# OmerShubi/DL_VQA

Measured on AMD Instinct MI355X. Metric: VQA samples/sec (train step), higher is better.
Workload: dtype f32; 1 GPU; VqaNet train step (fwd+softCE+bwd+Adam), batch 256/GPU, 224x224 images, 14-token questions, 1000-way head, train mode; global_batch=256, image_size=224, answers=1000, vocab=5000, parallelism=dp1

## Files before the change

dl_vqa_amd/_lib.py:

```python
from __future__ import annotations

import ctypes as C
import os

import torch

_HERE = os.path.dirname(os.path.abspath(__file__))
LIB_PATH = os.environ.get("VQA_LIB", os.path.join(_HERE, "libvqa_hip.so"))
HEADER_PATH = os.path.join(os.path.dirname(_HERE), "include", "vqa_hip.h")


def header_abi_version() -> int:
    import re
    with open(HEADER_PATH) as f:
        m = re.search(r"^#define\s+VQA_ABI_VERSION\s+(\d+)", f.read(), flags=re.M)
    if not m:
        raise VqaHipError(f"{HEADER_PATH}: no VQA_ABI_VERSION")
    return int(m.group(1))


f32p = C.c_void_p
u8p = C.c_void_p
i64p = C.c_void_p
i32, i64, f32, u64, vp = C.c_int, C.c_int64, C.c_float, C.c_uint64, C.c_void_p
# ... 86 lines not shown
    "vqa_preprocess_supported": (i32, [vp, vp, i64, i32, i32]),
    "vqa_preprocess_images": (i32, [u8p, i64, vp, vp, i64, vp, vp, i32, i32, vp, i32, vp, vp]),
    "vqa_f32_to_bf16": (i32, [f32p, vp, i64, vp]),
    "vqa_bf16_to_f32": (i32, [vp, f32p, i64, vp]),
    "vqa_dropout_to_bf16": (i32, [f32p, vp, i64, f32, u64, vp]),
    "vqa_f32_to_bf16_transpose": (i32, [f32p, vp, i32, i32, vp]),
    "vqa_gemm_bf16_workspace_bytes": (i64, [i32, i32, i32]),
    "vqa_gemm_bf16": (i32, [vp, i64, i32, vp, i64, i32, vp, i64, i32, i32, i32, i32, f32p, f32p,
                            f32p, i64, i32, i32, i32, i32, f32p, f32p, i64, i32, vp]),
    "vqa_gemm_plan": (i32, [i32, i32, i32, i32, i32, i32, i64, C.POINTER(i32), i32]),
    "vqa_gemm_tall_bf16_supported": (i32, [i32, i32, i32, i32, i32]),
    "vqa_gemm_tall_bf16_plan": (i32, [i32, i32, i32, C.POINTER(i32), i32]),
    "vqa_gemm_tall_bf16": (i32, [vp, i64, vp, i64, vp, i64, i32, i32, i32, f32p, i64, i32, i32, i32, i32, vp]),
    "vqa_conv_pack_weights_bf16": (i32, [f32p, vp, vp, i32, i32, i32, vp]),
    "vqa_conv3x3_relu_pool_fwd_bf16": (i32, [vp, vp, f32p, vp, i32, u8p, i32, i32, i32, i32, i32, i32, i32, vp]),
    "vqa_conv3x3_dgrad_bf16": (i32, [vp, u8p, vp, vp, i32, i32, i32, i32, i32, i32, i32, i32, vp]),
    "vqa_conv3x3_wgrad_bf16_workspace_bytes": (i64, [i32, i32, i32, i32, i32, i32]),
    "vqa_conv3x3_wgrad_bf16": (i32, [vp, vp, u8p, f32p, f32p, i32, i32, i32, i32, i32, i32, i32, f32p, i64, i32, vp]),
    "vqa_pconvf_supported": (i32, [i32, i32, i32, i32, i32]),
    "vqa_pconvf_weights_bytes": (i64, [i32, i32]),
    "vqa_pconvf_pack_weights": (i32, [f32p, f32p, i32, i32, vp]),
    "vqa_pconvf_dgrad": (i32, [f32p, u8p, f32p, f32p, i32, i32, i32, i32, i32, i32, vp]),
    "vqa_pconv_supported": (i32, [i32, i32, i32, i32, i32]),
    "vqa_pconv_weights_bytes": (i64, [i32, i32]),
    "vqa_pconv_pack_weights": (i32, [f32p, vp, vp, i32, i32, vp]),
    "vqa_pconv_fwd": (i32, [vp, vp, f32p, vp, i32, u8p, i32, i32, i32, i32, i32, i32, vp]),
    "vqa_pconv_wgrad_supported": (i32, [i32, i32, i32, i32]),
    "vqa_pconv_wgrad_workspace_bytes": (i64, [i32, i32, i32, i32, i32]),
    "vqa_pconv_wgrad": (i32, [vp, u8p, vp, f32p, f32p, i32, i32, i32, i32, i32, f32p, i64, i32, vp]),
    "vqa_pconv_dgrad": (i32, [vp, u8p, vp, vp, i32, i32, i32, i32, i32, i32, i32, vp]),
    "vqa_adam": (i32, [f32p, f32p, f32p, f32p, i64, f32, f32, f32, f32, i32, f32, vp]),
    "vqa_adam_segments": (i32, [f32p, f32p, f32p, f32p, i64, vp, i32, f32, vp]),
    "vqa_conv3x3_x3_plan": (i32, [i32, i32, i32, i32, i32, i32, i32, C.POINTER(i32), i32]),
}

K_GEMM, K_CONV_FWD, K_CONV_DGRAD, K_CONV_WGRAD = 0, 1, 2, 3
(K_L2NORM_FWD, K_L2NORM_BWD, K_ATT_SCORE_FWD, K_ATT_SCORE_BWD, K_ATT_APPLY_FWD, K_ATT_APPLY_BWD, K_ADAM, K_SOFTCE,
 K_DROPOUT, K_LSTM_SEQ, K_COUNT) = range(4, 15)


class LstmDir(C.Structure):
    _fields_ = [("w_hh", vp), ("xg", vp), ("gates", vp), ("Hs", vp), ("Cs", vp), ("c_final", vp),
                ("dgates", vp), ("dh", vp), ("dc", vp), ("reverse", i32)]


class AdamSegment(C.Structure):
    _fields_ = [("begin", i64), ("end", i64), ("lr", f32), ("beta1", f32), ("beta2", f32), ("eps", f32),
                ("weight_decay", f32), ("step", i32), ("decoupled", i32)]


ADAM_MAX_SEGMENTS = 64


class VqaHipError(RuntimeError):
    pass


_lib = None


def load() -> C.CDLL:
    global _lib
    if _lib is not None:
        return _lib
    if not os.path.exists(LIB_PATH):
        raise VqaHipError(
# ... 29 lines not shown
```

dl_vqa_amd/build.py:

```python
from __future__ import annotations

import os
import subprocess
import sys
from concurrent.futures import ThreadPoolExecutor

HERE = os.path.dirname(os.path.abspath(__file__))
CSRC = os.path.join(HERE, "csrc")
LIB = os.path.join(HERE, "libvqa_hip.so")
SOURCES = ([("gemm.hip", f"_p{k}", [f"-DVQA_GEMM_PART={k}"]) for k in (2, 3, 4, 5)]
           + [("gemm_x3.hip", f"_p{k}", [f"-DVQA_GEMM_PART={k}"]) for k in (1, 2, 3, 4)]
           + ["bf16.hip", ("gemm.hip", "_p1", ["-DVQA_GEMM_PART=1"]), "conv.hip", "conv_x3.hip", "conv_bf16.hip", "conv_patch_bf16.hip", "conv_patch_f32.hip", "gemm_tall_bf16.hip", "gemm.hip",
              "gemm_x3.hip", "runtime.hip", "conv0.hip", "conv0_dgrad.hip", "lstm.hip", "elementwise.hip", "conv_generic.hip", "att_score.hip", "topk.hip", "preprocess.hip"])
HEADERS = ["common.hpp", "gemm_core.hpp", "gemm_epilogue.hpp", "gemm_host.hpp", "bf16_core.hpp", "x3_core.hpp", "conv_device.inc", "conv_host.inc", "conv_bf16.inc", os.path.join("..", "..", "include", "vqa_hip.h")]
FLAGS = ["-O3", "--offload-arch=gfx950", "-fPIC", "-std=c++17", "-Wno-unused-result"]


def _hipcc() -> str:
    for cand in (os.environ.get("HIPCC"), "/opt/rocm/bin/hipcc", "hipcc"):
        if cand and (os.path.isabs(cand) and os.path.exists(cand) or not os.path.isabs(cand)):
            return cand
    return "hipcc"


def _stale(target: str, deps) -> bool:
    if not os.path.exists(target):
        return True
    t = os.path.getmtime(target)
    return any(os.path.getmtime(d) > t for d in deps if os.path.exists(d))


def _deps(src: str, seen=None) -> list:
    import re
    seen = set() if seen is None else seen
    out = []
    try:
        text = open(src).read()
    except OSError:
        return out
    for inc in re.findall(r'^\s*#\s*include\s+"([^"]+)"', text, flags=re.M):
        path = os.path.normpath(os.path.join(os.path.dirname(src), inc))
        if path not in seen and os.path.exists(path):
            seen.add(path)
            out.append(path)
            out += _deps(path, seen)
    return out
# ... 34 lines not shown
```

dl_vqa_amd/csrc/conv0.hip:

```cpp
#include "x3_core.hpp"

namespace vqa {

__host__ __device__ inline int c0_round_stride(int W, int want_mod) {
  int rs = W + 2;
  while (rs % 32 != want_mod) ++rs;
  return rs;
}

__device__ __forceinline__ float4 c0_load4(const void* x, int64_t e, int xh) {
  if (xh) {
    typedef _Float16 h16x4 __attribute__((ext_vector_type(4)));
    const h16x4 hv = *reinterpret_cast<const h16x4*>(static_cast<const uint16_t*>(x) + e);
    return make_float4((float)hv[0], (float)hv[1], (float)hv[2], (float)hv[3]);
  }
  return *reinterpret_cast<const float4*>(static_cast<const float*>(x) + e);
}

constexpr int C0_FR = 4;
constexpr int C0_PR = 2 * C0_FR + 2;

struct C0Tap { int c, ky, kx; };
__device__ __forceinline__ C0Tap c0_tap(int k) {
  const int c = k / 9, t = k - 9 * c, ky = t / 3;
// ... 644 lines not shown
#pragma unroll
      for (int j = 0; j < TN; ++j)
#pragma unroll
        for (int m = 0; m < 4; ++m) {
          const int o = (8 * g + 4 * h + m) * Co + 32 * j + l31;
          const uint32_t code = ams[o];
          const uint32_t dz = (uint32_t)dps[o] & ((code >> 2) - 1u);
          bsum[j] += __uint_as_float(dz << 16);
          const uint64_t f = (uint64_t)dz << ((code & 3u) * 16u);
          wlo[j][m] = (uint32_t)f;
          whi[j][m] = (uint32_t)(f >> 32);
        }
#pragma unroll
      for (int hs = 0; hs < 2; ++hs) {
        const bf16x8 af = __builtin_bit_cast(bf16x8, *reinterpret_cast<const uint4*>(arow + hs * RSTR + 32 * g));
#pragma unroll
        for (int j = 0; j < TN; ++j) {
          const bf16x8 bf = __builtin_bit_cast(bf16x8, hs ? make_uint4(whi[j][0], whi[j][1], whi[j][2], whi[j][3])
                                                          : make_uint4(wlo[j][0], wlo[j][1], wlo[j][2], wlo[j][3]));
          acc[j] = __builtin_amdgcn_mfma_f32_32x32x16_bf16(af, bf, acc[j], 0, 0, 0);
        }
      }
    }
  }
  c0_wgrad_write_slab<TN>(lds, acc, bsum, slab, bias_slab, tid, wave, l31, h);
}

__global__ void conv0_wgrad_reduce_kernel(const float* slab, const float* bias_slab, float* dw, float* dbias,
                                          int parts, int K, int Co) {
  __shared__ float red[256];
  const int k = blockIdx.x;
  const int co = threadIdx.x % Co, sl = threadIdx.x / Co, nsl = 256 / Co;
  float v = 0.f;
  if (sl < nsl)
    for (int p = sl; p < parts; p += nsl)
      v += (k < K) ? slab[((int64_t)p * 32 + k) * Co + co] : bias_slab[(int64_t)p * Co + co];
  red[threadIdx.x] = v;
  __syncthreads();
  if (sl == 0) {
    for (int s2 = 1; s2 < nsl; ++s2) v += red[s2 * Co + co];
    if (k < K) dw[(int64_t)co * K + k] = v; else dbias[co] = v;
  }
}

constexpr size_t kC0LdsMax = 160 * 1024;

static size_t c0_fwd_lds(int Ci, int W, int Co, bool wide_f32) {
  return (size_t)Ci * C0_PR * c0_round_stride(W, 16) * 4 + (wide_f32 ? (size_t)4 * 8 * Co * 5 : 0);
}
static int c0_c16_stride(int W) {
  int rs = W + 2;
  while (rs % 64 != 16) ++rs;
  return rs;
}
static size_t c0_fwd_c16_lds(int Ci, int W, int Co, int waves) {
  return (size_t)Ci * C0_PR * c0_c16_stride(W) * 2 + (size_t)waves * 8 * Co * 3 + (size_t)2 * (Co / 32) * 1024;
}
static int c0_wgrad_plane(int W) {
  int plane = 4 * c0_round_stride(W, 11);
  while (plane % 32 != 3) ++plane;
  return plane;
}
static size_t c0_combine_lds(int Co) { return (size_t)(4 * 32 + 4) * Co * 4; }
static size_t c0_wgrad_lds(int Ci, int W, int Co) {
  const size_t lds = (((size_t)Ci * c0_wgrad_plane(W) + 3) & ~(size_t)3) * 4 + (size_t)((W - 2) / 2) * Co * 5;
  return lds < c0_combine_lds(Co) ? c0_combine_lds(Co) : lds;
}
static size_t c0_wgrad_bf16_lds(int Ci, int RSTR, int NG, int Co) {
  const size_t lds = (size_t)3 * Ci * 4 * RSTR + (size_t)8 * NG * Co * 3;
// ... 145 lines not shown
```

dl_vqa_amd/csrc/elementwise.hip:

```cpp
#include <hip/hip_fp16.h>
#include "common.hpp"

namespace vqa {

__global__ void dropout_kernel(const float* x, float* y, int64_t n, float p, float inv_keep, uint64_t seed) {
  for (int64_t i = (int64_t)blockIdx.x * blockDim.x + threadIdx.x; i < n; i += (int64_t)gridDim.x * blockDim.x)
    y[i] = x[i] * drop_scale(seed, (uint64_t)i, p, inv_keep);
}

__global__ void dropout_add_kernel(const float* x, float* y, int64_t n, float p, float inv_keep, uint64_t seed) {
  const int64_t n4 = n / 4;
  for (int64_t i = (int64_t)blockIdx.x * blockDim.x + threadIdx.x; i < n4; i += (int64_t)gridDim.x * blockDim.x) {
    const float4 a = reinterpret_cast<const float4*>(x)[i];
    float4 b = reinterpret_cast<float4*>(y)[i];
    const float4 ds_ = drop_scale4(seed, (uint64_t)(4 * i), p, inv_keep);
    b.x += a.x * ds_.x; b.y += a.y * ds_.y; b.z += a.z * ds_.z; b.w += a.w * ds_.w;
    reinterpret_cast<float4*>(y)[i] = b;
  }
  if (blockIdx.x == 0 && threadIdx.x < n - 4 * n4) {
    const int64_t i = 4 * n4 + threadIdx.x;
    y[i] += x[i] * drop_scale(seed, (uint64_t)i, p, inv_keep);
  }
}

// ... 728 lines not shown
      float g = wsum * expf(row[i] - mx) * invs;
      for (int k = 0; k < kmax; ++k)
        if (a_idx[(int64_t)b * kmax + k] == (int64_t)i + 1) g -= (float)a_val[(int64_t)b * kmax + k] / 10.0f;
      d[i] = g * inv_batch;
    }
  }
}

__global__ void colsum_stage1(const float* x, int64_t ld, const uint8_t* mask, int64_t rows, int cols,
                              int64_t rows_per, float* slab) {
  __shared__ float part[4][64];
  const int cl = threadIdx.x & 63, rl = threadIdx.x >> 6;
  const int c = blockIdx.x * 64 + cl;
  const int64_t r0 = (int64_t)blockIdx.y * rows_per;
  const int64_t r1 = r0 + rows_per < rows ? r0 + rows_per : rows;
  float acc = 0.f;
  if (c < cols)
    for (int64_t r = r0 + rl; r < r1; r += 4) {
      const float v = x[r * ld + c];
      if (!mask || mask[r * cols + c] != 4) acc += v;
    }
  part[rl][cl] = acc;
  __syncthreads();
  if (rl == 0 && c < cols) slab[(int64_t)blockIdx.y * cols + c] = part[0][cl] + part[1][cl] + part[2][cl] + part[3][cl];
}
__global__ void colsum_stage2(const float* slab, int splits, int cols, float* out, int accumulate) {
  const int c = blockIdx.x * blockDim.x + threadIdx.x;
  if (c >= cols) return;
  float v = 0.f;
  for (int s = 0; s < splits; ++s) v += slab[(int64_t)s * cols + c];
  out[c] = accumulate ? out[c] + v : v;
}

static void colsum_plan(int64_t rows, int cols, int* splits, int64_t* rows_per) {
  const int ctiles = (cols + 63) / 64;
  int64_t s = (1024 + ctiles - 1) / ctiles;
  const int64_t max_s = (rows + 63) / 64;
  if (s > max_s) s = max_s;
  if (s < 1) s = 1;
  *rows_per = (rows + s - 1) / s;
  *splits = (int)((rows + *rows_per - 1) / *rows_per);
}
int64_t colsum_ws_bytes(int64_t rows, int cols) {
  int splits; int64_t rp;
  colsum_plan(rows, cols, &splits, &rp);
  return (int64_t)splits * cols * 4;
}
int colsum_launch(const float* x, int64_t ld, const uint8_t* mask, int64_t rows, int cols, float* out,
                  int accumulate, float* ws, int64_t ws_bytes, hipStream_t s) {
  int splits; int64_t rp;
  colsum_plan(rows, cols, &splits, &rp);
  if (!ws || ws_bytes < (int64_t)splits * cols * 4) {
    set_error("colsum: workspace %lld < %lld", (long long)ws_bytes, (long long)splits * cols * 4);
    return VQA_ERR_WORKSPACE;
  }
  hipLaunchKernelGGL(colsum_stage1, dim3((cols + 63) / 64, splits), dim3(256), 0, s, x, ld, mask, rows, cols, rp, ws);
  int rc = check_hip(hipGetLastError(), "colsum_stage1 launch");
  if (rc) return rc;
  hipLaunchKernelGGL(colsum_stage2, dim3((cols + 255) / 256), dim3(256), 0, s, ws, splits, cols, out, accumulate);
  return check_hip(hipGetLastError(), "colsum_stage2 launch");
}

__global__ __launch_bounds__(1024) void sum_bgp_kernel(const float* x, float* out, int B, int G, int P) {
  __shared__ float red[16];
  const int g = blockIdx.x;
  const int lane = threadIdx.x & 63, w = threadIdx.x >> 6;
  float s = 0.f;
// ... 571 lines not shown
```

dl_vqa_amd/csrc/gemm_core.hpp:

```cpp
#pragma once
#include <type_traits>
#include "common.hpp"

namespace vqa {

typedef float f32x16 __attribute__((ext_vector_type(16)));

#ifdef VQA_DIAG
static __device__ unsigned long long vqa_diag_buf[4];
static __device__ unsigned long long vqa_diag_ld[4];
#endif

#ifndef VQA_PRIO_MFMA
#define VQA_PRIO_MFMA 3
#endif
#ifndef VQA_EARLY_BARRIER
#define VQA_EARLY_BARRIER 2
#endif
#ifndef VQA_PF128
#define VQA_PF128 2
#endif
#ifndef VQA_PRIO_LOADER
#define VQA_PRIO_LOADER 0
#endif
// ... 567 lines not shown
}
template <class Cfg>
__device__ __forceinline__ int acc_col(int wn, int j, int lane) {
  return wn * Cfg::WN + 32 * j + (lane & 31);
}

template <class Cfg>
__device__ __forceinline__ void store_acc_tiles(f32x16 (&acc)[Cfg::TM][Cfg::TN], float* out, int64_t ld, int rows,
                                                int cols, int m0, int n0, int wm, int wn, int lane) {
  const bool interior = m0 + Cfg::BM <= rows && n0 + Cfg::BN <= cols;
  const uint32_t ldb = (uint32_t)ld * 4u;
  const uint32_t vl = (uint32_t)(4 * (lane >> 5)) * ldb + 4u * (uint32_t)(lane & 31);
  auto body = [&](auto inner) {
    constexpr bool INNER = decltype(inner)::value;
#pragma unroll
    for (int i = 0; i < Cfg::TM; ++i)
#pragma unroll
      for (int j = 0; j < Cfg::TN; ++j) {
        const int rowt = m0 + wm * Cfg::WM + 32 * i, colt = n0 + wn * Cfg::WN + 32 * j;
        const __amdgpu_buffer_rsrc_t rs = buf_rsrc(out + (int64_t)rowt * ld + colt);
        const bool cok = colt + (lane & 31) < cols;
#pragma unroll
        for (int r = 0; r < 16; ++r) {
          const int dr = (r & 3) + 8 * (r >> 2);
          const bool ok = INNER || (cok && rowt + 4 * (lane >> 5) + dr < rows);
          buf_store4(rs, acc[i][j][r], ok ? vl : BUF_OOB, (uint32_t)dr * ldb);
        }
      }
  };
  if (interior) body(std::true_type{}); else body(std::false_type{});
}

struct TileCoord { int mt, nt, split; };
__device__ __forceinline__ TileCoord tile_coord(int tiles_m, int tiles_n, int order = 0, int splits = 1) {
  const int t = xcd_swizzle(blockIdx.x, gridDim.x);
  const int tiles = tiles_m * tiles_n;
  TileCoord c;
  if (order == 1) {
    const int per_nt = tiles_m * splits;
    c.nt = t / per_nt;
    const int u = t - c.nt * per_nt;
    c.split = u / tiles_m;
    c.mt = u - c.split * tiles_m;
    return c;
  }
  c.split = t / tiles;
  const int u = t - c.split * tiles;
  c.mt = u / tiles_n;
  c.nt = u - c.mt * tiles_n;
  return c;
}

}
```

dl_vqa_amd/engine.py:

```python
from __future__ import annotations

import functools
import inspect
import os
from collections import namedtuple
from types import SimpleNamespace
from typing import Callable, Dict, Optional

import torch

from . import ops

Tensor = torch.Tensor

SITE_IMAGE, SITE_TEXT, SITE_ATT_V, SITE_ATT_Q, SITE_ATT_X, SITE_CLS1, SITE_CLS2 = 1, 2, 3, 4, 5, 6, 7
_MASK64 = (1 << 64) - 1


def _site_seed(base: int, site: int) -> int:
    return (base * 0x9E3779B97F4A7C15 + site * 0xD1B54A32D192ED03 + 0x632BE59BD9B4E019) & _MASK64


_SFX = ("", "_reverse")

# ... 492 lines not shown
                                                                   self.att_mode, ctx.p_att, sd(SITE_ATT_X))
        ops.colsum(dwx_part, n * NT, wx.numel(), Gr["attention.x_conv.weight"])
        dqp = new(B, mid)
        ops.sum_parts(dq_part, dqp, B, NT, mid)
        gx3 = self._x3_gemm(n * Pn)
        ops.gemm(dvprime, ctx.v_in, Gr["attention.v_conv.weight"], mid, C, n * Pn, transA=True, transB=False, lda=mid, ldb=C,
                 tag=44, x3=gx3)
        if encoded:
            dv_in = new(n * Pn, C)
            ops.gemm(dvprime, P["attention.v_conv.weight"], dv_in, n * Pn, C, mid, transB=False, lda=mid, ldb=C, tag=45, x3=gx3)
        self._q_lin_bwd(P, ctx, dqp, dcomb, Gr)
        ready("attention")

        def question_branch():
            self._question_bwd(P, ctx, dcomb, Gr)
            ready("text")

        if not encoded:
            question_branch()
            return None
        _, text_done = self._on_side_stream(dev, question_branch, backward=True)
        ops.dropout_add(dv_in, dvn, ctx.p_att, sd(SITE_ATT_V))
        dP = ops.l2norm_bwd(dvn, ctx.vn, ctx.norm, ctx.p_img, sd(SITE_IMAGE)).view_as(ctx.acts[-1])
        dv = self._conv_bwd(P, ctx, dP, Gr)
        ready("image")
        torch.cuda.current_stream(dev).wait_event(text_done)
        return dv

    @_device_current("dlogits")
    def backward(self, P: Dict[str, Tensor], ctx, dlogits: Tensor, Gr: Dict[str, Tensor],
                 on_ready: Optional[Callable[[str], None]] = None) -> Optional[Tensor]:
        dev = dlogits.device
        ready = on_ready if on_ready is not None else (lambda group: None)
        dcomb = self._classifier_bwd(P, ctx, dlogits, Gr)
        ready("classifier")
        dv_in = self._attention_bwd(P, ctx, dcomb, Gr)
        ready("attention")

        def question_branch():
            self._question_bwd(P, ctx, dcomb, Gr)
            ready("text")

        _, text_done = self._on_side_stream(dev, question_branch, backward=True)
        dv = self._image_bwd(P, ctx, dcomb, dv_in, Gr)
        ready("image")
        torch.cuda.current_stream(dev).wait_event(text_done)
        return dv

    def _classifier_bwd(self, P, ctx, dlogits, Gr):
        B, Dc, hid, A = ctx.B, self.Dc, self.hid, self.A
        dev = dlogits.device
        sd = lambda site: _site_seed(ctx.seed, site)
        if (A > 1 and dlogits.stride(1) != 1) or (B > 1 and dlogits.stride(0) < A):
            dlogits = dlogits.contiguous()
        ldA = (A + 3) // 4 * 4
        if ldA != A or not dlogits.is_contiguous() or dlogits.data_ptr() % 16:
            dl = torch.zeros(B, ldA, dtype=torch.float32, device=dev)
            ops.add2d(dlogits, dlogits.stride(0), None, 0, dl, ldA, B, A)
            dlogits = dl
        fc = ctx.fc
        if fc is not None:
            Bk, ld_dl, h_op, c_op, w2, w1 = fc.B8, A, fc.h16, fc.c16, fc.w2, fc.w1
        else:
            Bk, ld_dl, h_op, c_op, w2, w1 = B, ldA, ctx.h1d, ctx.c_in, P["classifier.lin2.weight"], P["classifier.lin1.weight"]
        dh1 = torch.empty(B, hid, dtype=torch.float32, device=dev)
        dcomb = torch.empty(B, Dc, dtype=torch.float32, device=dev)
        dl_op = self._fc_operand(fc, dlogits, ldA, A)
        _gemm(dl_op, h_op, Gr["classifier.lin2.weight"], A, hid, Bk, transA=True, transB=False, lda=ld_dl, ldb=hid, tag=40)
        ops.colsum(dlogits, B, A, Gr["classifier.lin2.bias"], ld=ldA)
        _gemm(dl_op, w2, dh1, B, hid, A, transB=False, lda=ld_dl, ldb=hid, tag=41)
        ops.relu_drop_bwd(ctx.h1, dh1, dh1, ctx.p_cls, sd(SITE_CLS2))
        dh_op = self._fc_operand(fc, dh1, hid, hid)
        _gemm(dh_op, c_op, Gr["classifier.lin1.weight"], hid, Dc, Bk, transA=True, transB=False, lda=hid, ldb=Dc, tag=42)
        ops.colsum(dh1, B, hid, Gr["classifier.lin1.bias"])
        _gemm(dh_op, w1, dcomb, B, Dc, hid, transB=False, lda=hid, ldb=Dc, tag=43)
        if ctx.p_cls > 0:
            ops.dropout(dcomb, ctx.p_cls, sd(SITE_CLS1), out=dcomb)
        return dcomb

    def _attention_bwd(self, P, ctx, dcomb, Gr):
        B, Pn = ctx.B, ctx.Pn
        G, C, mid, Dc, GC, Q = self.G, self.C, self.mid, self.Dc, self.GC, self.Q
        sd = lambda site: _site_seed(ctx.seed, site)
        new = lambda *shape: torch.empty(*shape, dtype=torch.float32, device=dcomb.device)
        ds_rows = new(B, G, 1)
        dscore, _ = ops.att_apply_bwd(dcomb, Dc, ctx.probs, ctx.vn, rowsum=ds_rows, want_dvn=False)
        ops.sum_bgp(ds_rows, Gr["attention.x_conv.bias"])
        wx = P["attention.x_conv.weight"].view(G, -1)
        dwx_part, dq_part, RS = ops.att_score_bwd(dscore, wx, ctx.xs, B, Pn, ctx.p_att, sd(SITE_ATT_X),
                                                  mode=self.att_mode, vprime=ctx.vprime, qp=ctx.qp)
        dxpre = ctx.xs
        ops.colsum(dwx_part, B * RS, wx.numel(), Gr["attention.x_conv.weight"])
        dqp = new(B, mid)
        ops.sum_parts(dq_part, dqp, B, RS, mid)
        v_op, wv_op = (ctx.v16.view(B * Pn, C), ctx.wv16) if self.bf16 else (ctx.v_in, P["attention.v_conv.weight"])
        gx3 = self._x3_gemm(B * Pn)
        _gemm(dxpre, v_op, Gr["attention.v_conv.weight"], mid, C, B * Pn, transA=True, transB=False, lda=mid, ldb=C, tag=44,
              x3=gx3)
        dv_in = new(B * Pn, C)
        _gemm(dxpre, wv_op, dv_in, B * Pn, C, mid, transB=False, lda=mid, ldb=C, tag=45, x3=gx3)
        self._q_lin_bwd(P, ctx, dqp, dcomb, Gr)
        return dv_in

    def _q_lin_bwd(self, P, ctx, dqp, dcomb, Gr):
        B = ctx.B
        mid, Dc, GC, Q = self.mid, self.Dc, self.GC, self.Q
        sd = lambda site: _site_seed(ctx.seed, site)
        new = lambda *shape: torch.empty(*shape, dtype=torch.float32, device=dcomb.device)
        ops.colsum(dqp, B, mid, Gr["attention.q_lin.bias"])
        fc = ctx.fc
        if fc is not None:
            Bk, q_op, ld_qop, wq = fc.B8, fc.q16, Q, fc.wq
        else:
            Bk, q_op, ld_qop, wq = B, ctx.q_in, ctx.ld_q, P["attention.q_lin.weight"]
        dqp_op = self._fc_operand(fc, dqp, mid, mid)
        _gemm(dqp_op, q_op, Gr["attention.q_lin.weight"], mid, Q, Bk, transA=True, transB=False, lda=mid, ldb=ld_qop, tag=46)
        direct = fc is None and ctx.p_att == 0
        dq_in, ld_dq = (dcomb[:, GC:], Dc) if direct else (new(B, Q), Q)
        _gemm(dqp_op, wq, dq_in, B, Q, mid, transB=False, lda=mid, ldb=Q, ldc=ld_dq, accumulate=direct, tag=47)
        if not direct:
            if ctx.p_att > 0:
                ops.dropout(dq_in, ctx.p_att, sd(SITE_ATT_Q), out=dq_in)
            ops.add2d(dcomb[:, GC:], Dc, dq_in, Q, dcomb[:, GC:], Dc, B, Q)

    def _question_bwd(self, P, ctx, dcomb, Gr):
        B, T = ctx.B, ctx.T
        E, H, Dc, GC = self.E, self.H, self.Dc, self.GC
        dev = dcomb.device
        new = lambda *shape: torch.empty(*shape, dtype=torch.float32, device=dev)
        dirs = []
        for d, st in enumerate(ctx.lstm):
            dc = new(B, H)
            ops.add2d(dcomb[:, GC + d * H:], Dc, None, 0, dc, H, B, H)
            dh = torch.zeros(B, H, dtype=torch.float32, device=dev)
            st["dgates"] = new(T, B, 4 * H)
            dirs.append(dict(w_hh=P["text.lstm.weight_hh_l0" + _SFX[d]], gates=st["gates"], Hs=st["Hs"], Cs=st["Cs"],
                             dgates=st["dgates"], dh=dh, dc=dc, reverse=bool(d)))
        fused, use_graph = self._lstm_schedule()
        if fused:
            ops.lstm_seq_bwd(dirs, ctx.q_len, B, T, H, use_graph=use_graph)
        else:
            for st in dirs:
                for n, (t, si, so) in enumerate(reversed(self._lstm_steps(T, st["reverse"]))):
                    ops.lstm_cell_bwd(st["gates"][t], st["Cs"][si], st["Cs"][so], ctx.q_len, t, st["dh"], st["dc"],
                                      st["dgates"][t])
                    if n != T - 1:
                        ops.gemm(st["dgates"][t], st["w_hh"], st["dh"], B, H, 4 * H, transB=False, lda=4 * H, ldb=H,
                                 accumulate=True, tag=50)
        l16 = ctx.x16 is not None
        x_op, Ek = (ctx.x16, ctx.x16.shape[1]) if l16 else (ctx.x_emb, E)
        dx_parts = []
        for d, st in enumerate(ctx.lstm):
# ... 65 lines not shown
```

dl_vqa_amd/ops.py:

```python
from __future__ import annotations

from typing import Optional, Tuple

import torch

from . import _lib
from ._lib import call, ptr, stream

_ws = {}


def workspace(nbytes: int, device) -> torch.Tensor:
    key = (str(device), torch.cuda.current_stream(device).cuda_stream)
    t = _ws.get(key)
    if t is None or t.numel() * 4 < nbytes:
        t = torch.empty(_workspace_floats(nbytes), dtype=torch.float32, device=device)
        _ws[key] = t
    return t


def _workspace_floats(nbytes: int) -> int:
    return max(nbytes // 4 + 1024, 1 << 20)


def _chk(t: torch.Tensor, dtype=torch.float32):
    assert t.is_cuda and t.dtype == dtype, (t.device, t.dtype)


def _gemm(name: str, c_kind: tuple, A, B, C, M, N, K, transA, transB, lda, ldb, ldc, bias1, bias2, rowgroup, rg_div, rg_op, relu,
          accumulate, aux, tag) -> torch.Tensor:
    lib = _lib.load()
    lda = lda if lda is not None else (M if transA else K)
    ldb = ldb if ldb is not None else (K if transB else N)
    ldc = ldc if ldc is not None else N
    nbytes = getattr(lib, name + "_workspace_bytes")(M, N, K)
    ws = workspace(nbytes, A.device) if nbytes else None
    call(name, ptr(A), lda, int(transA), ptr(B), ldb, int(transB), ptr(C), ldc, *c_kind, M, N, K,
         ptr(bias1), ptr(bias2), ptr(rowgroup), (rowgroup.stride(0) if rowgroup is not None else 0),
         rg_div, rg_op, int(relu), int(accumulate), ptr(aux), ptr(ws), (ws.numel() * 4 if ws is not None else 0),
         tag, stream())
    return C


def gemm(A: torch.Tensor, B: torch.Tensor, C: torch.Tensor, M: int, N: int, K: int, *, transA=False,
         transB=True, lda=None, ldb=None, ldc=None, bias1=None, bias2=None, rowgroup=None, rg_div=1,
         rg_op=0, relu=False, accumulate=False, aux=None, tag=0, x3=False) -> torch.Tensor:
    return _gemm("vqa_gemm_x3" if x3 else "vqa_gemm", (), A, B, C, M, N, K, transA, transB, lda, ldb, ldc, bias1, bias2, rowgroup,
                 rg_div, rg_op, relu, accumulate, aux, tag)


GEMM_ENGINES = {"vqa_gemm": 0, "vqa_gemm_x3": 1, "vqa_gemm_bf16": 2}
GEMM_PLAN_FIELDS = ("BM", "BN", "tiles_m", "tiles_n", "nk", "splits", "ks_per_split", "order", "persistent", "wide")


def gemm_plan(engine: str, M: int, N: int, K: int, *, transA=False, transB=True, workspace_bytes=None) -> dict:
    import ctypes
    lib = _lib.load()
    if workspace_bytes is None:
        nbytes = getattr(lib, engine + "_workspace_bytes")(M, N, K) if min(M, N, K) > 0 else 0
        workspace_bytes = _workspace_floats(nbytes) * 4 if nbytes else 0
    out = (ctypes.c_int32 * len(GEMM_PLAN_FIELDS))()
    call("vqa_gemm_plan", GEMM_ENGINES[engine], M, N, K, int(transA), int(transB), workspace_bytes, out, len(out))
    return dict(zip(GEMM_PLAN_FIELDS, out))


def nchw_to_nhwc4(x: torch.Tensor) -> torch.Tensor:
    B, Cc, H, W = x.shape
    y = torch.empty(B, H, W, 4, dtype=torch.float32, device=x.device)
    call("vqa_nchw_to_nhwc4", ptr(x), ptr(y), B, Cc, H, W, stream())
    return y


def conv_pack_weights(w: torch.Tensor, CiP: int, need_wd: bool = True):
    Co, Ci = w.shape[0], w.shape[1]
    wf = torch.empty(9 * CiP, Co, dtype=torch.float32, device=w.device)
    wd = torch.empty(9 * Co, CiP, dtype=torch.float32, device=w.device) if need_wd else None
    call("vqa_conv_pack_weights", ptr(w), ptr(wf), ptr(wd), Co, Ci, CiP, stream())
    return wf, wd


def conv_out_hw(H: int, W: int, stride: int) -> Tuple[int, int]:
# ... 815 lines not shown
```

include/vqa_hip.h:

```cpp
#ifndef VQA_HIP_H
#define VQA_HIP_H

#include <stdint.h>

#ifdef __cplusplus
extern "C" {
#endif

#define VQA_ABI_VERSION 9

#define VQA_OK 0
#define VQA_ERR_INVALID 1
#define VQA_ERR_HIP 2
#define VQA_ERR_WORKSPACE 3

typedef void* vqa_stream_t;

int vqa_abi_version(void);
const char* vqa_last_error(void);
int vqa_device_ok(void);

int vqa_reload_knobs(void);

enum {
// ... 241 lines not shown
int vqa_conv3x3_dgrad_x3(const void* dpooled, int dp_packed, const uint8_t* argmax, const void* wd_planes, float* dx, int B,
                         int H, int W, int CiP, int Co, int stride, int tag, vqa_stream_t stream);
int64_t vqa_conv3x3_wgrad_x3_workspace_bytes(int B, int H, int W, int CiP, int Co, int stride);
int64_t vqa_x3_pack_pooled_grad_workspace_bytes(int Co);
int vqa_x3_pack_pooled_grad(const float* dpooled, const uint8_t* argmax, void* packed, float* dbias, int64_t windows, int Co,
                            float* workspace, int64_t workspace_bytes, vqa_stream_t stream);
int vqa_conv3x3_wgrad_x3(const void* x, int x_packed, const float* dpooled, const void* dpooled_packed,
                         const uint8_t* argmax, float* dw, float* dbias, int B, int H, int W, int CiP, int Ci, int Co,
                         int stride, float* workspace, int64_t workspace_bytes, int tag, vqa_stream_t stream);

int64_t vqa_gemm_x3_workspace_bytes(int M, int N, int K);
int vqa_gemm_x3(const float* A, int64_t lda, int transA, const float* B, int64_t ldb, int transB, float* C, int64_t ldc,
                int M, int N, int K, const float* bias1, const float* bias2, const float* rowgroup, int64_t rg_ld,
                int rg_div, int rg_op, int relu, int accumulate, float* aux, float* workspace, int64_t workspace_bytes,
                int tag, vqa_stream_t stream);

int vqa_adam(float* param, const float* grad, float* exp_avg, float* exp_avg_sq, int64_t n, float lr,
             float beta1, float beta2, float eps, int step, float grad_scale, vqa_stream_t stream);

#define VQA_ADAM_MAX_SEGMENTS 64
#define VQA_ADAM_SEGMENTS_MAX_BLOCKS 2048
typedef struct {
  int64_t begin, end;
  float lr, beta1, beta2, eps, weight_decay;
  int step;
  int decoupled;
} vqa_adam_segment;
int vqa_adam_segments(float* param, const float* grad, float* exp_avg, float* exp_avg_sq, int64_t n,
                      const vqa_adam_segment* segs , int n_segs, float grad_scale,
                      vqa_stream_t stream);

int vqa_conv3x3_x3_plan(int pass, int B, int H, int W, int CiP, int Co, int stride, int32_t* out, int n_out);

#ifdef __cplusplus
}
#endif
#endif
```

Before: 9898 samples/s.

## Fuse FC backward dX, dW and bias reductions into one kernel launch

Result: no change. 9862 samples/s (-0.4%).

```diff
diff --git a/dl_vqa_amd/_lib.py b/dl_vqa_amd/_lib.py
--- a/dl_vqa_amd/_lib.py
+++ b/dl_vqa_amd/_lib.py
@@ -142,6 +142,7 @@
     "vqa_adam": (i32, [f32p, f32p, f32p, f32p, i64, f32, f32, f32, f32, i32, f32, vp]),
     "vqa_adam_segments": (i32, [f32p, f32p, f32p, f32p, i64, vp, i32, f32, vp]),
     "vqa_conv3x3_x3_plan": (i32, [i32, i32, i32, i32, i32, i32, i32, C.POINTER(i32), i32]),
+    "vqa_fc_bwd": (i32, [f32p, i64, f32p, i64, f32p, i64, f32p, i64, i32, f32p, i64, f32p, i32, i32, i32, i32, vp]),
 }
 
 K_GEMM, K_CONV_FWD, K_CONV_DGRAD, K_CONV_WGRAD = 0, 1, 2, 3
diff --git a/dl_vqa_amd/build.py b/dl_vqa_amd/build.py
--- a/dl_vqa_amd/build.py
+++ b/dl_vqa_amd/build.py
@@ -11,7 +11,7 @@
 SOURCES = ([("gemm.hip", f"_p{k}", [f"-DVQA_GEMM_PART={k}"]) for k in (2, 3, 4, 5)]
            + [("gemm_x3.hip", f"_p{k}", [f"-DVQA_GEMM_PART={k}"]) for k in (1, 2, 3, 4)]
            + ["bf16.hip", ("gemm.hip", "_p1", ["-DVQA_GEMM_PART=1"]), "conv.hip", "conv_x3.hip", "conv_bf16.hip", "conv_patch_bf16.hip", "conv_patch_f32.hip", "gemm_tall_bf16.hip", "gemm.hip",
-              "gemm_x3.hip", "runtime.hip", "conv0.hip", "conv0_dgrad.hip", "lstm.hip", "elementwise.hip", "conv_generic.hip", "att_score.hip", "topk.hip", "preprocess.hip"])
+              "gemm_x3.hip", "runtime.hip", "conv0.hip", "conv0_dgrad.hip", "lstm.hip", "elementwise.hip", "conv_generic.hip", "att_score.hip", "topk.hip", "preprocess.hip", "fc_bwd.hip"])
 HEADERS = ["common.hpp", "gemm_core.hpp", "gemm_epilogue.hpp", "gemm_host.hpp", "bf16_core.hpp", "x3_core.hpp", "conv_device.inc", "conv_host.inc", "conv_bf16.inc", os.path.join("..", "..", "include", "vqa_hip.h")]
 FLAGS = ["-O3", "--offload-arch=gfx950", "-fPIC", "-std=c++17", "-Wno-unused-result"]
 
diff --git a/dl_vqa_amd/csrc/conv0.hip b/dl_vqa_amd/csrc/conv0.hip
--- a/dl_vqa_amd/csrc/conv0.hip
+++ b/dl_vqa_amd/csrc/conv0.hip
@@ -700,9 +700,20 @@
   const int k = blockIdx.x;
   const int co = threadIdx.x % Co, sl = threadIdx.x / Co, nsl = 256 / Co;
   float v = 0.f;
-  if (sl < nsl)
-    for (int p = sl; p < parts; p += nsl)
-      v += (k < K) ? slab[((int64_t)p * 32 + k) * Co + co] : bias_slab[(int64_t)p * Co + co];
+  if (sl < nsl) {
+    constexpr int U = 24;
+    const float* src = (k < K) ? slab + (int64_t)k * Co + co : bias_slab + co;
+    const int64_t step = (k < K) ? (int64_t)32 * Co : Co;
+    int p = sl;
+    for (; p + (U - 1) * nsl < parts; p += U * nsl) {
+      float t[U];
+#pragma unroll
+      for (int j = 0; j < U; ++j) t[j] = src[(int64_t)(p + j * nsl) * step];
+#pragma unroll
+      for (int j = 0; j < U; ++j) v += t[j];
+    }
+    for (; p < parts; p += nsl) v += src[(int64_t)p * step];
+  }
   red[threadIdx.x] = v;
   __syncthreads();
   if (sl == 0) {
diff --git a/dl_vqa_amd/csrc/elementwise.hip b/dl_vqa_amd/csrc/elementwise.hip
--- a/dl_vqa_amd/csrc/elementwise.hip
+++ b/dl_vqa_amd/csrc/elementwise.hip
@@ -784,7 +784,7 @@
   out[c] = accumulate ? out[c] + v : v;
 }
 
-static void colsum_plan(int64_t rows, int cols, int* splits, int64_t* rows_per) {
+void colsum_plan(int64_t rows, int cols, int* splits, int64_t* rows_per) {
   const int ctiles = (cols + 63) / 64;
   int64_t s = (1024 + ctiles - 1) / ctiles;
   const int64_t max_s = (rows + 63) / 64;
diff --git a/dl_vqa_amd/csrc/fc_bwd.hip b/dl_vqa_amd/csrc/fc_bwd.hip
--- /dev/null
+++ b/dl_vqa_amd/csrc/fc_bwd.hip
@@ -0,0 +1,129 @@
+#include "gemm_host.hpp"
+
+namespace vqa {
+
+void colsum_plan(int64_t rows, int cols, int* splits, int64_t* rows_per);
+
+using Cfg64 = TileCfg<64, 64, 2, 2>;
+using AR64 = PlainR<Cfg64::NVA, Cfg64::LT>;
+using AC64 = PlainC<Cfg64::NVA, Cfg64::LT>;
+using BC64 = PlainC<Cfg64::NVB, Cfg64::LT>;
+constexpr int FC_SMEM_BYTES = SmemLayout<Cfg64, true, false>::BYTES > SmemLayout<Cfg64, false, false>::BYTES
+                                  ? SmemLayout<Cfg64, true, false>::BYTES : SmemLayout<Cfg64, false, false>::BYTES;
+static_assert(Cfg64::TM == 1 && Cfg64::TN == 1, "one MFMA tile per wave: a chain is one f32x16");
+
+struct FcProduct {
+  const float* A; int64_t lda;
+  const float* B; int64_t ldb;
+  EpiParams pe;
+  int K, tiles_m, tiles_n, nk, splits, ks_per_split, order;
+};
+struct FcBias { const float* dy; int64_t ld; int rows, cols, splits; int64_t rows_per; float* out; };
+
+template <class AL, class BL>
+__device__ __forceinline__ void fc_product(const FcProduct& g, int t, float* smem) {
+  const int lane = threadIdx.x & 63, wave = threadIdx.x >> 6;
+  const int wm = wave / Cfg64::WAVES_N, wn = wave % Cfg64::WAVES_N;
+  const TileCoord tc = tile_coord_of(t, g.tiles_m, g.tiles_n, g.order, 1);
+  const int m0 = tc.mt * Cfg64::BM, n0 = tc.nt * Cfg64::BN;
+  const typename AL::Params pa{g.A, g.lda, g.pe.M, g.K};
+  const typename BL::Params pb{g.B, g.ldb, g.pe.N, g.K};
+  const bool four = g.pe.N % 4 == 0;
+  const int chains = g.splits == 1 ? 1 : four ? 4 : 1, stride = four ? 4 : 1;
+  f32x16 acc[1][1], cur, keep, low;
+#pragma unroll
+  for (int r = 0; r < 16; ++r) cur[r] = keep[r] = low[r] = 0.f;
+  bool mfma = false;
+  for (int c = 0; c < chains; ++c) {
+#pragma unroll
+    for (int r = 0; r < 16; ++r) cur[r] = 0.f;
+    for (int s = c; s < g.splits; s += stride) {
+      const int ks0 = s * g.ks_per_split;
+      const int ks1 = min(g.nk, ks0 + g.ks_per_split);
+      acc_zero<Cfg64>(acc);
+      mfma = gemm_mainloop<Cfg64, AL, BL>(
+          [&](AL& al, BL& bl) {
+            al.init(pa, m0, loader_tid<Cfg64>(), ks0);
+            bl.init(pb, n0, loader_tid<Cfg64>(), ks0);
+          },
+          [](AL&, BL&) {}, acc, ks0, ks1, g.K, smem);
+      if (mfma && g.splits > 1) cur += acc[0][0];
+    }
+    if (c == 1) low = keep + cur;
+    else if (c != 3) keep = cur;
+  }
+  if (!mfma) return;
+  if (g.splits > 1) acc[0][0] = four ? low + (keep + cur) : cur;
+  if (g.pe.accumulate) gemm_epilogue_mode<Cfg64, 0, true, false>(g.pe, acc, m0, n0, wm, wn, lane);
+  else gemm_epilogue_mode<Cfg64, 0, false, false>(g.pe, acc, m0, n0, wm, wn, lane);
+}
+
+__device__ __forceinline__ void fc_bias(const FcBias& b, int blk, float* smem) {
+  float (*part)[64] = reinterpret_cast<float (*)[64]>(smem);
+  const int cl = threadIdx.x & 63, rl = threadIdx.x >> 6;
+  const int c = blk * 64 + cl;
+  const bool on = rl < 4 && c < b.cols;
+  float total = 0.f;
+  for (int s = 0; s < b.splits; ++s) {
+    const int64_t r0 = (int64_t)s * b.rows_per;
+    const int64_t r1 = r0 + b.rows_per < b.rows ? r0 + b.rows_per : b.rows;
+    float acc = 0.f;
+    if (on)
+      for (int64_t r = r0 + rl; r < r1; r += 4) acc += b.dy[r * b.ld + c];
+    if (rl < 4) part[rl][cl] = acc;
+    __syncthreads();
+    if (on && rl == 0) total += part[0][cl] + part[1][cl] + part[2][cl] + part[3][cl];
+    __syncthreads();
+  }
+  if (on && rl == 0) b.out[c] = total;
+}
+
+__global__ __launch_bounds__(Cfg64::THREADS, Cfg64::MIN_WAVES) void fc_bwd_kernel(FcProduct dx, FcProduct dw, FcBias db, int n_dx,
+                                                                                   int n_dw) {
+  extern __shared__ __attribute__((aligned(16))) float smem[];
+  const int bid = blockIdx.x;
+  if (bid < n_dx) return fc_product<AR64, BC64>(dx, xcd_swizzle(bid, n_dx), smem);
+  if (bid < n_dx + n_dw) return fc_product<AC64, BC64>(dw, xcd_swizzle(bid - n_dx, n_dw), smem);
+  fc_bias(db, bid - n_dx - n_dw, smem);
+}
+
+static FcProduct fc_product_of(const float* A, int64_t lda, const float* B, int64_t ldb, float* C, int64_t ldc, int M, int N, int K,
+                               int accumulate) {
+  const GemmPlan p = plan_gemm(M, N, K);
+  const int tm = (M + 63) / 64, tn = (N + 63) / 64;
+  FcProduct g{A, lda, B, ldb, epi_params(C, nullptr, ldc, M, N, nullptr, nullptr, nullptr, 0, 1, 0, 0, accumulate, nullptr),
+              K, tm, tn, p.nk, p.splits, p.ks_per_split, (tm <= 8 && tn >= 16 && knobs().weight_stationary != 0) ? 1 : 0};
+  g.pe.slab = nullptr;
+#ifdef VQA_DIAG
+  g.pe.bar_dbg = nullptr;
+#endif
+  return g;
+}
+
+}
+
+using namespace vqa;
+
+extern "C" {
+
+int vqa_fc_bwd(const float* dY, int64_t ldy, const float* X, int64_t ldx, const float* W, int64_t ldw, float* dX, int64_t ldc,
+               int accumulate, float* dW, int64_t lddw, float* db, int B, int N, int K, int tag, vqa_stream_t stream) {
+  if (int rc = check_gemm_args("vqa_fc_bwd", 4, dY, ldy, W, ldw, dX, ldc, B, K, N, nullptr, 0)) return rc;
+  if (int rc = check_gemm_args("vqa_fc_bwd", 4, dY, ldy, X, ldx, dW, lddw, N, K, B, nullptr, 0)) return rc;
+  VQA_REQUIRE(db, "vqa_fc_bwd: null operand");
+  VQA_REQUIRE(ldy >= N && ldx >= K && ldw >= K && ldc >= K && lddw >= K,
+              "vqa_fc_bwd: a leading dimension is below its row length (ldy=%lld ldx=%lld ldw=%lld ldc=%lld lddw=%lld)",
+              (long long)ldy, (long long)ldx, (long long)ldw, (long long)ldc, (long long)lddw);
+  hipStream_t s = (hipStream_t)stream;
+  const FcProduct gx = fc_product_of(dY, ldy, W, ldw, dX, ldc, B, K, N, accumulate);
+  const FcProduct gw = fc_product_of(dY, ldy, X, ldx, dW, lddw, N, K, B, 0);
+  FcBias gb{dY, ldy, B, N, 1, B, db};
+  colsum_plan(B, N, &gb.splits, &gb.rows_per);
+  const int n_dx = gx.tiles_m * gx.tiles_n, n_dw = gw.tiles_m * gw.tiles_n;
+  set_launch_tag(tag);
+  ProfScope prof(VQA_K_GEMM, s);
+  return launch_kernel(fc_bwd_kernel, KernelNames{"hipFuncSetAttribute(fc_bwd)", "fc_bwd_kernel launch"},
+                       dim3(n_dx + n_dw + (N + 63) / 64), Cfg64::THREADS, FC_SMEM_BYTES, s, gx, gw, gb, n_dx, n_dw);
+}
+
+}
diff --git a/dl_vqa_amd/csrc/gemm_core.hpp b/dl_vqa_amd/csrc/gemm_core.hpp
--- a/dl_vqa_amd/csrc/gemm_core.hpp
+++ b/dl_vqa_amd/csrc/gemm_core.hpp
@@ -623,8 +623,7 @@
 }
 
 struct TileCoord { int mt, nt, split; };
-__device__ __forceinline__ TileCoord tile_coord(int tiles_m, int tiles_n, int order = 0, int splits = 1) {
-  const int t = xcd_swizzle(blockIdx.x, gridDim.x);
+__device__ __forceinline__ TileCoord tile_coord_of(int t, int tiles_m, int tiles_n, int order, int splits) {
   const int tiles = tiles_m * tiles_n;
   TileCoord c;
   if (order == 1) {
@@ -641,5 +640,8 @@
   c.nt = u - c.mt * tiles_n;
   return c;
 }
-
-}
+__device__ __forceinline__ TileCoord tile_coord(int tiles_m, int tiles_n, int order = 0, int splits = 1) {
+  return tile_coord_of(xcd_swizzle(blockIdx.x, gridDim.x), tiles_m, tiles_n, order, splits);
+}
+
+}
diff --git a/dl_vqa_amd/engine.py b/dl_vqa_amd/engine.py
--- a/dl_vqa_amd/engine.py
+++ b/dl_vqa_amd/engine.py
@@ -548,7 +548,7 @@
                  on_ready: Optional[Callable[[str], None]] = None) -> Optional[Tensor]:
         dev = dlogits.device
         ready = on_ready if on_ready is not None else (lambda group: None)
-        dcomb = self._classifier_bwd(P, ctx, dlogits, Gr)
+        dcomb = self._classifier_bwd(P, ctx, dlogits, Gr, one_launch=True)
         ready("classifier")
         dv_in = self._attention_bwd(P, ctx, dcomb, Gr)
         ready("attention")
@@ -563,7 +563,7 @@
         torch.cuda.current_stream(dev).wait_event(text_done)
         return dv
 
-    def _classifier_bwd(self, P, ctx, dlogits, Gr):
+    def _classifier_bwd(self, P, ctx, dlogits, Gr, one_launch=False):
         B, Dc, hid, A = ctx.B, self.Dc, self.hid, self.A
         dev = dlogits.device
         sd = lambda site: _site_seed(ctx.seed, site)
@@ -581,6 +581,13 @@
             Bk, ld_dl, h_op, c_op, w2, w1 = B, ldA, ctx.h1d, ctx.c_in, P["classifier.lin2.weight"], P["classifier.lin1.weight"]
         dh1 = torch.empty(B, hid, dtype=torch.float32, device=dev)
         dcomb = torch.empty(B, Dc, dtype=torch.float32, device=dev)
+        if one_launch and fc is None:
+            ops.fc_bwd(dlogits, h_op, w2, dh1, Gr["classifier.lin2.weight"], Gr["classifier.lin2.bias"], B, A, hid, ldy=ldA, tag=40)
+            ops.relu_drop_bwd(ctx.h1, dh1, dh1, ctx.p_cls, sd(SITE_CLS2))
+            ops.fc_bwd(dh1, c_op, w1, dcomb, Gr["classifier.lin1.weight"], Gr["classifier.lin1.bias"], B, hid, Dc, tag=42)
+            if ctx.p_cls > 0:
+                ops.dropout(dcomb, ctx.p_cls, sd(SITE_CLS1), out=dcomb)
+            return dcomb
         dl_op = self._fc_operand(fc, dlogits, ldA, A)
         _gemm(dl_op, h_op, Gr["classifier.lin2.weight"], A, hid, Bk, transA=True, transB=False, lda=ld_dl, ldb=hid, tag=40)
         ops.colsum(dlogits, B, A, Gr["classifier.lin2.bias"], ld=ldA)
@@ -615,25 +622,32 @@
               x3=gx3)
         dv_in = new(B * Pn, C)
         _gemm(dxpre, wv_op, dv_in, B * Pn, C, mid, transB=False, lda=mid, ldb=C, tag=45, x3=gx3)
-        self._q_lin_bwd(P, ctx, dqp, dcomb, Gr)
+        self._q_lin_bwd(P, ctx, dqp, dcomb, Gr, one_launch=True)
         return dv_in
 
-    def _q_lin_bwd(self, P, ctx, dqp, dcomb, Gr):
+    def _q_lin_bwd(self, P, ctx, dqp, dcomb, Gr, one_launch=False):
         B = ctx.B
         mid, Dc, GC, Q = self.mid, self.Dc, self.GC, self.Q
         sd = lambda site: _site_seed(ctx.seed, site)
         new = lambda *shape: torch.empty(*shape, dtype=torch.float32, device=dcomb.device)
-        ops.colsum(dqp, B, mid, Gr["attention.q_lin.bias"])
         fc = ctx.fc
+        one_launch = one_launch and fc is None
+        if not one_launch:
+            ops.colsum(dqp, B, mid, Gr["attention.q_lin.bias"])
         if fc is not None:
             Bk, q_op, ld_qop, wq = fc.B8, fc.q16, Q, fc.wq
         else:
             Bk, q_op, ld_qop, wq = B, ctx.q_in, ctx.ld_q, P["attention.q_lin.weight"]
         dqp_op = self._fc_operand(fc, dqp, mid, mid)
-        _gemm(dqp_op, q_op, Gr["attention.q_lin.weight"], mid, Q, Bk, transA=True, transB=False, lda=mid, ldb=ld_qop, tag=46)
+        if not one_launch:
+            _gemm(dqp_op, q_op, Gr["attention.q_lin.weight"], mid, Q, Bk, transA=True, transB=False, lda=mid, ldb=ld_qop, tag=46)
         direct = fc is None and ctx.p_att == 0
         dq_in, ld_dq = (dcomb[:, GC:], Dc) if direct else (new(B, Q), Q)
-        _gemm(dqp_op, wq, dq_in, B, Q, mid, transB=False, lda=mid, ldb=Q, ldc=ld_dq, accumulate=direct, tag=47)
+        if one_launch:
+            ops.fc_bwd(dqp, q_op, wq, dq_in, Gr["attention.q_lin.weight"], Gr["attention.q_lin.bias"], B, mid, Q, ldx=ld_qop,
+                       ldc=ld_dq, accumulate=direct, tag=46)
+        else:
+            _gemm(dqp_op, wq, dq_in, B, Q, mid, transB=False, lda=mid, ldb=Q, ldc=ld_dq, accumulate=direct, tag=47)
         if not direct:
             if ctx.p_att > 0:
                 ops.dropout(dq_in, ctx.p_att, sd(SITE_ATT_Q), out=dq_in)
diff --git a/dl_vqa_amd/ops.py b/dl_vqa_amd/ops.py
--- a/dl_vqa_amd/ops.py
+++ b/dl_vqa_amd/ops.py
@@ -47,6 +47,14 @@
          rg_op=0, relu=False, accumulate=False, aux=None, tag=0, x3=False) -> torch.Tensor:
     return _gemm("vqa_gemm_x3" if x3 else "vqa_gemm", (), A, B, C, M, N, K, transA, transB, lda, ldb, ldc, bias1, bias2, rowgroup,
                  rg_div, rg_op, relu, accumulate, aux, tag)
+
+
+def fc_bwd(dY: torch.Tensor, X: torch.Tensor, W: torch.Tensor, dX: torch.Tensor, dW: torch.Tensor, db: torch.Tensor,
+           B: int, N: int, K: int, *, ldy=None, ldx=None, ldw=None, ldc=None, lddw=None, accumulate=False, tag=0) -> torch.Tensor:
+    call("vqa_fc_bwd", ptr(dY), ldy if ldy is not None else N, ptr(X), ldx if ldx is not None else K,
+         ptr(W), ldw if ldw is not None else K, ptr(dX), ldc if ldc is not None else K, int(accumulate),
+         ptr(dW), lddw if lddw is not None else K, ptr(db), B, N, K, tag, stream())
+    return dX
 
 
 GEMM_ENGINES = {"vqa_gemm": 0, "vqa_gemm_x3": 1, "vqa_gemm_bf16": 2}
diff --git a/include/vqa_hip.h b/include/vqa_hip.h
--- a/include/vqa_hip.h
+++ b/include/vqa_hip.h
@@ -297,6 +297,10 @@
 
 int vqa_conv3x3_x3_plan(int pass, int B, int H, int W, int CiP, int Co, int stride, int32_t* out, int n_out);
 
+int vqa_fc_bwd(const float* dY, int64_t ldy, const float* X, int64_t ldx, const float* W, int64_t ldw,
+               float* dX, int64_t ldc, int accumulate, float* dW, int64_t lddw, float* db, int B, int N, int K,
+               int tag, vqa_stream_t stream);
+
 #ifdef __cplusplus
 }
 #endif
```
